# bruniss/multi-task-3d-resencoder-unet

Hardware: AMD Instinct MI355X
Metric: train patches/sec (b,c,z,y,x) ResEncM 1x128^3 (higher is better)
Workload: dtype bf16; 1 GPU; cfg2: ResEncM (6 stages, feats [32, 64, 128, 256, 512, 512], blocks [1, 3, 4, 6, 6, 6]), 1-in, heads ['sheet'], patch 128x128x128, batch 2/GPU, full train step (fwd+loss+bwd+allreduce+clip+AdamW); global_batch=2, parallelism=dp1

## Files before the change

include/rxunet.h:

```cpp
#ifndef RXUNET_H
#define RXUNET_H

#include <stddef.h>
#include <stdint.h>

#ifdef __cplusplus
extern "C" {
#endif

#define RX_OK 0
#define RX_EINVAL (-1)
#define RX_EUNSUPPORTED (-2)
#define RX_ELAUNCH (-3)
#define RX_EWORKSPACE (-4)

typedef enum { RX_F32 = 0, RX_BF16 = 1, RX_F16 = 2 } rx_dtype;
typedef enum { RX_ACT_NONE = 0, RX_ACT_SIGMOID = 1, RX_ACT_SOFTMAX = 2 } rx_head_act;

typedef struct {
  void* ptr;
  int32_t n, z, y, x, c, ld;
  int64_t cs;
} rx_act;

// ... 10 lines not shown
                  const int* taps, void* const* w_fwd, void* const* w_bwd, void* stream);

size_t rx_conv_workspace_hint(void);
int rx_conv3d_fwd(rx_dtype dt, const rx_act* x, const void* w_fwd, const float* bias, const rx_act* y,
                  const int32_t kernel[3], const int32_t stride[3], void* ws, size_t ws_bytes, void* stream);
int rx_conv3d_fwd_stats(rx_dtype dt, const rx_act* x, const void* w_fwd, const float* bias, const rx_act* y,
                        const int32_t kernel[3], const int32_t stride[3], float eps, float* stats, void* ws,
                        size_t ws_bytes, void* stream);
int rx_conv3d_bwd_data(rx_dtype dt, const rx_act* dy, const void* w_bwd, const rx_act* dx,
                       const int32_t kernel[3], const int32_t stride[3], int accumulate, void* ws,
                       size_t ws_bytes, void* stream);
int rx_conv3d_bwd_data_instats(rx_dtype dt, const rx_act* dy, const void* w_bwd, const rx_act* dx,
                               const int32_t kernel[3], const int32_t stride[3], int accumulate, const rx_act* in_y,
                               const float* in_stats, float slope, float* m12, int* fused, void* ws, size_t ws_bytes,
                               void* stream);
size_t rx_conv3d_bwd_weight_workspace(const rx_act* x, const rx_act* dy, const int32_t kernel[3]);
int rx_conv3d_bwd_weight(rx_dtype dt, const rx_act* x, const rx_act* dy, float* dw, const int32_t kernel[3],
                         const int32_t stride[3], void* ws, size_t ws_bytes, void* stream);

int rx_convT3d_fwd(rx_dtype dt, const rx_act* x, const void* w_fwd, const float* bias, const rx_act* y,
                   const int32_t stride[3], void* ws, size_t ws_bytes, void* stream);
int rx_convT3d_bwd_data(rx_dtype dt, const rx_act* dy, const void* w_bwd, const rx_act* dx,
                        const int32_t stride[3], int accumulate, void* ws, size_t ws_bytes, void* stream);
size_t rx_convT3d_bwd_weight_workspace(const rx_act* x, const rx_act* dy, const int32_t stride[3]);
int rx_convT3d_bwd_weight(rx_dtype dt, const rx_act* x, const rx_act* dy, float* dw, const int32_t stride[3],
                          void* ws, size_t ws_bytes, void* stream);

size_t rx_instnorm_stats_workspace(const rx_act* y);
int rx_instnorm_stats(rx_dtype dt, const rx_act* y, float eps, float* stats, void* ws, size_t ws_bytes,
                      void* stream);
// ... 183 lines not shown
```

multi-task-3d-resencoder-unet_amd/csrc/rx_common.h:

```cpp
#pragma once
#include <hip/hip_runtime.h>
#include <type_traits>
#include <stdint.h>
#include <stdio.h>
#include <stdlib.h>
#include <string.h>

#include "../../include/rxunet.h"

hipError_t rx_func_attr_once(const void* fn, hipFuncAttribute attr, int value);
#ifndef RX_NO_HOST_MACROS
#define hipFuncSetAttribute(fn, attr, value) rx_func_attr_once((fn), (attr), (value))
#endif

inline int rx_env_mask(const char* name) {
  const char* e = getenv(name);
  return e ? atoi(e) : 0;
}

#define RX_WAVE 64

typedef __bf16 bf16_t;
typedef _Float16 f16_t;
typedef float f32x4 __attribute__((ext_vector_type(4)));
// ... 22 lines not shown
  } while (0)

#ifndef RX_ST16
#define RX_ST16 1
#endif
__device__ inline u32x4 rx_pair16(u32x2 a, u32x2 b) {
  auto r0 = __builtin_amdgcn_permlane32_swap(a[0], b[0], false, false);
  auto r1 = __builtin_amdgcn_permlane32_swap(a[1], b[1], false, false);
  return u32x4{r0[0], r1[0], r0[1], r1[1]};
}

struct RxBwdStat {
  const rx_act* y;
  const float* stats;
  float slope;
};

#ifndef RX_ABLATION
#define RX_ABLATION 0
#endif
#define RX_ABLATE(g, bit) (RX_ABLATION && ((g).dbg & (bit)))

template <typename T>
struct Elem;
template <>
struct Elem<float> {
  static constexpr int PER16 = 4;
  __device__ static inline float to_f(float v) { return v; }
  __device__ static inline float from_f(float v) { return v; }
};
// ... 174 lines not shown
```

multi-task-3d-resencoder-unet_amd/csrc/rx_conv_halo.hip:

```cpp
#include <stdlib.h>

#include <type_traits>

#include "rx_common.h"
#include "rx_internal.h"

struct ConvHaloGeom {
  int N, Z, Y, X;
  int Ci, Co, ldi, ldo;
  long in_ss, out_ss;
  long in_cs, out_cs;
  int TZ, TY, TX, lTX, lTY;
  int HY, HX, HV, VT;
  int tz_n, ty_n, tx_n, NT;
  int order;
  int wgs_s;
  float* stat_part;
  const void* bs_y;
  const float* bs_stats;
  int bs_ldy;
  long bs_yss;
  float bs_slope;
  int accumulate, flip, dbg;
};

#define RX_CH_MAX_HV 656
#define RX_CH_XPIECES ((RX_CH_MAX_HV * 4 + 255) / 256)

__device__ inline int hswz(int row, int chunk) { return row * 4 + (chunk ^ ((row >> 2) & 3)); }

__device__ inline int lane_voxel(int l ) {
  return l < 4 ? l : l < 12 ? l + 12 : l < 16 ? l - 8 : l < 20 ? l + 8 : l < 28 ? l - 12 : l;
}

template <typename T, int BN>
__global__ __launch_bounds__(256, 2) void conv_halo_kernel(const T* __restrict__ in, const T* __restrict__ w, const float* __restrict__ bias,
                                                           T* __restrict__ out, const ConvHaloGeom g) {
// ... 540 lines not shown
        if (RX_ST16) {
#pragma unroll
          for (int pr = 0; pr < 2; ++pr)
            *reinterpret_cast<u32x4*>(op + 16 * pr + 8 * fh) = rx_pair16(piece[2 * pr], piece[2 * pr + 1]);
        }
      }
      lds_only_barrier();
    }
    if (STATS || BS) ch_stat_flush<1>(s1, s2, g.stat_part, sn, g.wgs_s * 4, sl * 4 + wave, g.Co, 0, lane);
  }
}

#define CH64_W_BYTES (9 * 64 * 64)
#define CH64_X_BYTES (648 * 64)

template <typename T, bool FLIP, bool XDMA = false, bool STATS = false, bool ACC = false, bool BSP = false, int NA = 2>
__global__ __launch_bounds__(512, 1) void conv_halo64ws_kernel(const T* __restrict__ in, const T* __restrict__ w, const float* __restrict__ bias,
                                                               T* __restrict__ out, const ConvHaloGeom g, int tiles_per_wg) {
  constexpr int P = Elem<T>::PER16;
  constexpr int KB = 4 * P;
  constexpr int TZ = 4, TY = 4, TX = 16, HY = TY + 2, HX = TX + 2, HV = 648;
  constexpr int XPIECES = (HV * 4 + 255) / 256;
  static_assert(NA == 2 || (XDMA && !BSP), "32-channel blocks: LDS-DMA variants without backward sums only");
  constexpr int BNW = 32 * NA;
  constexpr int W_BYTES = 9 * BNW * 64;
  constexpr int WINSTR = 9 * BNW / 16;
  constexpr int WPIECES = (WINSTR + 3) / 4;
  constexpr int CENTRE = HY * HX + HX + 1;
  extern __shared__ __attribute__((aligned(16))) unsigned char smem[];
  unsigned char* sWb = smem;
  unsigned char* sXb = smem + 2 * W_BYTES;

  const int tid = threadIdx.x, lane = tid & 63;
  const int wave = __builtin_amdgcn_readfirstlane(tid >> 6);
  const int lid = g.order ? rx_xcd_remap(blockIdx.y * gridDim.x + blockIdx.x, gridDim.x * gridDim.y) : blockIdx.x * gridDim.y + blockIdx.y;
  const int vb = lid / gridDim.y;
  int t_begin = vb * tiles_per_wg, t_end = min(g.NT, t_begin + tiles_per_wg);
  const int NTs = g.NT / g.N;
// ... 81 lines not shown
      }
    };
    auto commit_phase = [&](int ph) {
      if (ph % 3 == 0) {
        unsigned char* sX = sXb + ((ph / 3) & 1) * CH64_X_BYTES;
#pragma unroll
        for (int p = 0; p < XPIECES; ++p) {
          const int row = (ptid >> 2) + 64 * p;
          if (xh[p] >= 0) *reinterpret_cast<u32x4*>(sX + row * 64 + ((chunk ^ ((row >> 2) & 3)) << 4)) = xr[p];
        }
      }
    };
    if (XDMA) {
      const int bc = ptid & 7, bvg = ptid >> 3;
      float bs1[8], bs2[8], bmean[8];
      u32x4 yv[8];
      if (BSP) {
#pragma unroll
        for (int j = 0; j < 8; ++j) bs1[j] = 0.f, bs2[j] = 0.f, bmean[j] = g.bs_stats[2 * ((size_t)sn * g.Co + n0 + 8 * bc + j)];
      }
      auto bs_load_y = [&](int tile) {
        int n, z0, y0, x0;
        tile_origin(tile, n, z0, y0, x0);
        const T* yp = (const T*)g.bs_y + (long)n * g.bs_yss + n0 + 8 * bc;
#pragma unroll
        for (int p = 0; p < 8; ++p) {
          const int v = bvg + 32 * p;
          const int z = z0 + (v >> 6), y = y0 + ((v >> 4) & 3), x = x0 + (v & 15);
          yv[p] = (z < g.Z && y < g.Y && x < g.X) ? *reinterpret_cast<const u32x4*>(yp + ((long)(z * g.Y + y) * g.X + x) * g.bs_ldy) : u32x4{0u, 0u, 0u, 0u};
        }
      };
      auto bs_accumulate = [&](int tile, const unsigned char* sS) {
        int n, z0, y0, x0;
        tile_origin(tile, n, z0, y0, x0);
#pragma unroll
        for (int p = 0; p < 8; ++p) {
          const int v = bvg + 32 * p;
          const int z = z0 + (v >> 6), y = y0 + ((v >> 4) & 3), x = x0 + (v & 15);
          if (z < g.Z && y < g.Y && x < g.X) {
            const u32x4 gq = *reinterpret_cast<const u32x4*>(sS + v * 144 + bc * 16);
#pragma unroll
            for (int j = 0; j < 8; ++j) {
              float gg = Elem<T>::to_f(reinterpret_cast<const T*>(&gq)[j]);
              const float yc = Elem<T>::to_f(reinterpret_cast<const T*>(&yv[p])[j]) - bmean[j];
              if (!(yc > 0.f)) gg *= g.bs_slope;
              bs1[j] += gg;
              bs2[j] += gg * yc;
            }
          }
        }
      };
      if (nphase > 0) {
        dma_weights(0);
        dma_halo(0);
        asm volatile("s_waitcnt vmcnt(0)" ::: "memory");
      }
      lds_only_barrier();
      int pit = 0, pending = -1;
      const unsigned char* pendS = nullptr;
      for (int ph = 0; ph < nphase; ++ph) {
        const bool tile_end = pit == ppt - 1;
        if (ph + 1 < nphase) {
          dma_weights(ph + 1);
          if (ph + 2 < nphase && (ph + 2) % 3 == 0) {
            dma_halo(ph + 2);
            if (pw == 0)
              asm volatile("s_waitcnt vmcnt(11)" ::: "memory");
            else
              asm volatile("s_waitcnt vmcnt(10)" ::: "memory");
          } else {
            if (BSP && pending >= 0) {
              bs_accumulate(pending, pendS);
              pending = -1;
            }
            if (BSP && tile_end) bs_load_y(t_begin + ph / ppt);
            asm volatile("s_waitcnt vmcnt(0)" ::: "memory");
          }
        } else if (BSP) {
          bs_load_y(t_begin + ph / ppt);
          asm volatile("s_waitcnt vmcnt(0)" ::: "memory");
        }
        lds_only_barrier();
        if (++pit == ppt) {
          pit = 0;
          if (BSP) {
            lds_only_barrier();
            pending = t_begin + ph / ppt;
            pendS = sXb + ((ph / 3) & 1) * CH64_X_BYTES;
          }
        }
      }
      if (BSP) {
        if (pending >= 0) bs_accumulate(pending, pendS);
#pragma unroll
        for (int j = 0; j < 8; ++j) {
          float u = bs1[j], v = bs2[j];
#pragma unroll
          for (int o = 8; o < 64; o <<= 1) {
            u += __shfl_xor(u, o, 64);
            v += __shfl_xor(v, o, 64);
          }
          bs1[j] = u, bs2[j] = v;
        }
        if (pl < 8) {
          float* p0 = g.stat_part + ((size_t)(sn * (g.wgs_s * 4) + sl * 4 + pw) * 2) * g.Co + n0 + 8 * pl;
#pragma unroll
          for (int j = 0; j < 8; ++j) p0[j] = bs1[j], p0[g.Co + j] = bs2[j];
        }
// ... 154 lines not shown
                else if (decltype(RA)::value) f += Elem<T>::to_f(reinterpret_cast<const T*>(&old2)[i]);
                vals[i] = Elem<T>::from_f(f);
                if (STATS) {
                  const float r = Elem<T>::to_f(vals[i]);
                  s1[a][4 * g4 + i] += r;
                  s2[a][4 * g4 + i] += r * r;
                }
              }
              if (BSP) *reinterpret_cast<u32x2*>(sS + v * SROW + co * 2) = *reinterpret_cast<u32x2*>(vals);
              else if (!RX_ABLATE(g, 16) || vals[0] == (T)12345.f) *reinterpret_cast<u32x2*>(op + cm) = *reinterpret_cast<u32x2*>(vals);
            }
        };
        RX_EPI_DISPATCH(bias != nullptr, !ACC && g.accumulate != 0, epi);
      }
      lds_only_barrier();
      if (BSP) {
        int t2 = tid;
        asm volatile("" : "+v"(t2));
        const int ry = t2 >> 7, rx = (t2 >> 3) & 15, c = t2 & 7;
        T* gp = out + (long)n * g.out_ss + ((long)(z0 * g.Y + y0 + ry) * g.X + x0 + rx) * g.ldo + n0 + (c >> 2) * g.out_cs + (c & 3) * 8;
        const unsigned char* lp = sS + (t2 >> 3) * SROW + c * 16;
        const bool okx = x0 + rx < g.X;
#pragma unroll
        for (int p = 0; p < 8; ++p) {
          const int zz = p >> 1, yy = 2 * (p & 1);
          if (okx && z0 + zz < g.Z && y0 + ry + yy < g.Y)
            *reinterpret_cast<u32x4*>(gp + ((long)(zz * g.Y + yy) * g.X) * g.ldo) = *reinterpret_cast<const u32x4*>(lp + p * 32 * SROW);
        }
      }
      ++ph;
    }
// ... 13 lines not shown
  const int per = (NTs + wgs_s - 1) / wgs_s;
  wgs_s = (NTs + per - 1) / per;
  wgs = wgs_s * g.N;
  const_cast<ConvHaloGeom&>(g).wgs_s = wgs_s;
  dim3 grid(wgs, cob);
#define RX_64WS(...)                                                                                                                   \
  do {                                                                                                                                 \
    (void)hipFuncSetAttribute(reinterpret_cast<const void*>(&conv_halo64ws_kernel<T, __VA_ARGS__>), hipFuncAttributeMaxDynamicSharedMemorySize, (int)lds); \
    hipLaunchKernelGGL((conv_halo64ws_kernel<T, __VA_ARGS__>), grid, dim3(512), lds, st, (const T*)in, (const T*)w, bias, (T*)out, g, per); \
  } while (0)
  const bool dma_ok = (long)g.N * g.in_ss * 2 < 0x7fffff00L;
  if (dma_ok && g.stat_part && !g.flip && !g.bs_y) {
    RX_64WS(false, true, true);
    return;
  }
  if (dma_ok && g.bs_y && g.stat_part && g.flip && !((uintptr_t)out & 15) && g.ldo % 8 == 0 && g.out_cs % 8 == 0 && !((uintptr_t)g.bs_y & 15) &&
      g.bs_ldy % 8 == 0) {
    if (g.accumulate) RX_64WS(true, true, false, true, true);
    else RX_64WS(true, true, false, false, true);
    return;
  }
  const_cast<ConvHaloGeom&>(g).bs_y = nullptr;
  const_cast<ConvHaloGeom&>(g).stat_part = nullptr;
  if (dma_ok && g.accumulate && g.flip) RX_64WS(true, true, false, true);
  else if (dma_ok && g.flip) RX_64WS(true, true);
  else if (dma_ok) RX_64WS(false, true);
  else if (g.flip) RX_64WS(true, false);
  else RX_64WS(false, false);
#undef RX_64WS
}

template <typename T>
static bool ch32ws_launch(hipStream_t st, const void* in, const void* w, const float* bias, void* out, const ConvHaloGeom& g) {
  const size_t lds = (size_t)2 * (9 * 32 * 64 + CH64_X_BYTES);
// ... 128 lines not shown
  g.tz_n = (g.Z + TZ - 1) / TZ, g.ty_n = (g.Y + TY - 1) / TY, g.tx_n = (g.X + TX - 1) / TX;
  g.NT = g.N * g.tz_n * g.ty_n * g.tx_n;
  g.accumulate = accumulate, g.flip = flip;
  g.order = 1;
  static const int dbg = rx_env_mask("RX_DBG");
  g.dbg = dbg;
  int BN = (g.Co % 64 == 0) ? 64 : 32;
  if (BN == 64 && (long)g.NT * (g.Co / 64) < 256) BN = 32;
  if ((in->cs || out->cs) && (long)g.NT * (g.Co / BN) < 192) RX_FAIL(RX_EUNSUPPORTED, "conv_halo: planar-concat operand on a layer too small for the halo kernels");
  if ((long)g.NT * (g.Co / BN) < 192) return 0;
  dim3 grid(g.NT, g.Co / BN);
  if (BN == 32 && TZ == 4 && TY == 4 && TX == 16 && dt != RX_F32 && g.Ci == 32 && g.Co == 32 && g.NT >= 512) {
    rx_note_kernel("conv_halo32p_kernel");
    if (in->cs || out->cs) RX_FAIL(RX_EUNSUPPORTED, "conv_halo32p: planar-concat operand");
    const bool room = stat_part && stat_chunks && (size_t)g.N * 1024 * 2 * g.Co * sizeof(float) <= stat_bytes;
    const bool fuse32 = room && ((!flip && !accumulate && !bs) || (flip && bs));
    g.stat_part = fuse32 ? stat_part : nullptr;
    if (fuse32 && bs) {
      g.bs_y = bs->y->ptr, g.bs_ldy = bs->y->ld, g.bs_yss = rx_act_voxels(bs->y) * (long)bs->y->ld;
      g.bs_stats = bs->stats, g.bs_slope = bs->slope;
    }
    if (dt == RX_BF16)
      ch32p_launch<bf16_t>(st, in->ptr, w, bias, out->ptr, g);
    else
      ch32p_launch<f16_t>(st, in->ptr, w, bias, out->ptr, g);
    hipError_t e4 = hipGetLastError();
    if (e4 != hipSuccess) {
      rx_set_error("conv_halo32p: %s", hipGetErrorString(e4));
      return RX_ELAUNCH;
    }
    if (fuse32) *stat_chunks = g.wgs_s * 4;
// ... 39 lines not shown
      return RX_ELAUNCH;
    }
    if (fuse32n) *stat_chunks = NTs32 * 4;
    return 1;
  }
  if (g.Co % 64 == 0 && TZ == 4 && TY == 4 && TX == 16 && dt != RX_F32 && (long)g.NT * (g.Co / 64) >= 256) {
    if (in->cs) RX_FAIL(RX_EUNSUPPORTED, "conv_halo64ws: planar-concat input");
    rx_note_kernel("conv_halo64ws_kernel");
    const bool room64 = stat_part && stat_chunks && (size_t)g.N * 1024 * 2 * g.Co * sizeof(float) <= stat_bytes;
    const bool fuse64 = room64 && !flip && !accumulate && !bs;
    const bool fuse64b = room64 && flip && bs;
    g.stat_part = (fuse64 || fuse64b) ? stat_part : nullptr;
    if (fuse64b) {
      g.bs_y = bs->y->ptr, g.bs_ldy = bs->y->ld, g.bs_yss = rx_act_voxels(bs->y) * (long)bs->y->ld;
      g.bs_stats = bs->stats, g.bs_slope = bs->slope;
    }
    if (dt == RX_BF16)
      ch64ws_launch<bf16_t>(st, in->ptr, w, bias, out->ptr, g);
    else
      ch64ws_launch<f16_t>(st, in->ptr, w, bias, out->ptr, g);
    hipError_t e5 = hipGetLastError();
    if (e5 != hipSuccess) {
      rx_set_error("conv_halo64ws: %s", hipGetErrorString(e5));
      return RX_ELAUNCH;
    }
    if (fuse64 && g.stat_part) *stat_chunks = g.wgs_s * 4;
    if (fuse64b && g.bs_y && g.stat_part) *stat_chunks = g.wgs_s * 4;
    g.stat_part = nullptr, g.bs_y = nullptr;
    return 1;
  }
// ... 16 lines not shown
```

multi-task-3d-resencoder-unet_amd/csrc/rx_igemm.hip:

```cpp
#include <stdlib.h>

#include "rx_common.h"
#include "rx_internal.h"


struct IgemmPhase {
  int Qz, Qy, Qx, Vq;
  int opz, opy, opx;
  int tap0, ntaps;
  int mtile0, mtiles;
  long slab_off;
};

struct IgemmGeom {
  int Zi, Yi, Xi, Ci, ldi;
  long in_ss;
  int isz, isy, isx;
  int Zo, Yo, Xo, Co, ldo;
  long out_ss;
  int osz, osy, osx;
  int accumulate, ksplit, nph, total_mtiles;
  IgemmPhase ph[8];
  RxTap taps[RX_MAX_TAPS];
};
// ... 530 lines not shown
    RxBwdStat bs{in_y, in_stats, slope};
    int chunks = 0;
    rc = rx_conv_halo_try(dt, dy, w_bwd, nullptr, dx, 1, accumulate, (hipStream_t)stream, (float*)ws, wsb, &chunks, &bs);
    if (rc < 0) return rc;
    if (rc == 1) {
      if (chunks > 0) {
        rx_inbwd_fused_finalize_launch((const float*)ws, dx->n, chunks, dx->c, (double)rx_act_voxels(dx), in_stats, m12, (hipStream_t)stream);
        hipError_t e = hipGetLastError();
        if (e != hipSuccess) RX_FAIL(RX_ELAUNCH, "rx_conv3d_bwd_data_instats(finalize): %s", hipGetErrorString(e));
        *fused = 1;
      }
      return RX_OK;
    }
  }
  return rx_conv3d_bwd_data(dt, dy, w_bwd, dx, kernel, stride, accumulate, ws, wsb, stream);
}

extern "C" int rx_conv3d_fwd_stats(rx_dtype dt, const rx_act* x, const void* w_fwd, const float* bias, const rx_act* y,
                                   const int32_t kernel[3], const int32_t stride[3], float eps, float* stats, void* ws, size_t wsb,
                                   void* stream) {
  RX_RECORD(stream, [=, x_ = RxActV(x), y_ = RxActV(y), kernel_ = RxI3V(kernel), stride_ = RxI3V(stride)](void* s) { return rx_conv3d_fwd_stats(dt, x_.p(), w_fwd, bias, y_.p(), kernel_.v, stride_.v, eps, stats, ws, wsb, s); });
  if (!rx_act_ok_planar(x) || !rx_act_ok(y) || !w_fwd || !stats || !ws) RX_FAIL(RX_EINVAL, "rx_conv3d_fwd_stats: bad arguments");
  int rc = check13(kernel, stride, "rx_conv3d_fwd_stats");
  if (rc) return rc;
  if (is_333_s1(kernel, stride) && y->n == x->n && y->z == x->z && y->y == x->y && y->x == x->x) {
    int chunks = 0;
    rc = rx_conv_halo_try(dt, x, w_fwd, bias, y, 0, 0, (hipStream_t)stream, (float*)ws, wsb, &chunks, nullptr);
    if (rc < 0) return rc;
    if (rc == 1 && chunks > 0) {
      rx_stats_finalize_launch((const float*)ws, y->n, chunks, y->c, (double)rx_act_voxels(y), eps, stats, (hipStream_t)stream);
// ... 171 lines not shown
```

multi-task-3d-resencoder-unet_amd/engine/lib.py:

```python
import ctypes
import os
from ctypes import POINTER, c_char_p, c_double, c_float, c_int, c_int32, c_long, c_size_t, c_void_p

import torch

_HERE = os.path.dirname(os.path.abspath(__file__))
LIB_PATH = os.environ.get("RX_LIBRARY") or os.path.join(os.path.dirname(_HERE), "csrc", "librxunet.so")

RX_F32, RX_BF16, RX_F16 = 0, 1, 2
RX_ACT_NONE, RX_ACT_SIGMOID, RX_ACT_SOFTMAX = 0, 1, 2
DTYPE_CODE = {torch.float32: RX_F32, torch.bfloat16: RX_BF16, torch.float16: RX_F16}
RX_SW_U8, RX_SW_U16, RX_SW_F32 = 0, 1, 2
RX_SW_SCALE, RX_SW_ZSCORE = 0, 1
RX_SW_BLEND_AVERAGE, RX_SW_BLEND_UNIT, RX_SW_BLEND_NONE = 0, 1, 2
RX_SW_CAST_U8, RX_SW_CAST_U16 = 0, 1
RX_AUG_PW_NONE, RX_AUG_PW_AFFINE, RX_AUG_PW_PLANE, RX_AUG_PW_NOISE = 0, 1, 2, 3
RX_AUG_G3_NONE, RX_AUG_G3_FILTER, RX_AUG_G3_DOWNSCALE = 0, 1, 2
RX_AUG_MAX_K, RX_AUG_MAX_BOXES = 21, 4
RX_LOSS_BCE_LOGITS, RX_LOSS_BCE_PROB, RX_LOSS_MSE = 0, 1, 2
RX_REDUCE_MEAN, RX_REDUCE_SUM = 0, 1


class RxError(RuntimeError):
    pass
# ... 15 lines not shown

_SIGNATURES = {
    "rx_abi_version": (c_int, []),
    "rx_last_error": (c_char_p, []),
    "rx_device_arch_ok": (c_int, []),
    "rx_last_conv_kernel": (c_char_p, []),
    "rx_pack_conv_weight": (c_int, [c_int, c_void_p, c_int, c_int, c_int, c_void_p, c_void_p, c_void_p]),
    "rx_pack_convT_weight": (c_int, [c_int, c_void_p, c_int, c_int, c_int, c_void_p, c_void_p, c_void_p]),
    "rx_pack_multi": (c_int, [c_int, c_int, c_void_p, c_void_p, c_void_p, c_void_p, c_void_p, c_void_p, c_void_p, c_void_p]),
    "rx_conv_workspace_hint": (c_size_t, []),
    "rx_conv3d_fwd": (c_int, [c_int, _P, c_void_p, c_void_p, _P, I3, I3, c_void_p, c_size_t, c_void_p]),
    "rx_conv3d_fwd_stats": (c_int, [c_int, _P, c_void_p, c_void_p, _P, I3, I3, c_float, c_void_p, c_void_p, c_size_t, c_void_p]),
    "rx_conv3d_bwd_data": (c_int, [c_int, _P, c_void_p, _P, I3, I3, c_int, c_void_p, c_size_t, c_void_p]),
    "rx_conv3d_bwd_data_instats": (c_int, [c_int, _P, c_void_p, _P, I3, I3, c_int, _P, c_void_p, c_float, c_void_p, POINTER(c_int),
                                           c_void_p, c_size_t, c_void_p]),
    "rx_instnorm_act_bwd_apply": (c_int, [c_int, _P, _P, c_void_p, _P, c_float, c_void_p, _P, _P, c_int, c_void_p]),
    "rx_conv3d_bwd_weight_workspace": (c_size_t, [_P, _P, I3]),
    "rx_conv3d_bwd_weight": (c_int, [c_int, _P, _P, c_void_p, I3, I3, c_void_p, c_size_t, c_void_p]),
    "rx_convT3d_fwd": (c_int, [c_int, _P, c_void_p, c_void_p, _P, I3, c_void_p, c_size_t, c_void_p]),
    "rx_convT3d_bwd_data": (c_int, [c_int, _P, c_void_p, _P, I3, c_int, c_void_p, c_size_t, c_void_p]),
    "rx_convT3d_bwd_weight_workspace": (c_size_t, [_P, _P, I3]),
    "rx_convT3d_bwd_weight": (c_int, [c_int, _P, _P, c_void_p, I3, c_void_p, c_size_t, c_void_p]),
    "rx_instnorm_stats_workspace": (c_size_t, [_P]),
    "rx_instnorm_stats": (c_int, [c_int, _P, c_float, c_void_p, c_void_p, c_size_t, c_void_p]),
    "rx_instnorm_act_fwd": (c_int, [c_int, _P, c_void_p, _P, _P, c_float, c_void_p]),
    "rx_instnorm_stats_mask": (c_int, [c_void_p, c_void_p, c_int, c_void_p]),
    "rx_instnorm_fwd": (c_int, [c_int, _P, c_float, c_void_p, _P, _P, c_float, c_void_p, c_size_t, c_void_p]),
    "rx_instnorm_act_bwd": (c_int, [c_int, _P, _P, c_void_p, _P, c_float, _P, _P, c_int, c_void_p, c_size_t,
                                    c_void_p]),
    "rx_instnorm_act_bwd_res": (c_int, [c_int, _P, _P, c_void_p, _P, c_float, _P, I3, _P, _P, c_void_p, c_size_t, c_void_p]),
# ... 132 lines not shown
```

multi-task-3d-resencoder-unet_amd/engine/ops.py:

```python
from ctypes import byref, c_void_p

import numpy as np
import torch

from . import lib as _l
from .lib import I3, RxAct, check, load, stream_ptr

_WS = {}
_PROF = None


def set_profiler(p):
    global _PROF
    _PROF = p


class LaunchProfiler:

    def __init__(self):
        self.pending = []
        self.groups = {}
        self.pending_hbm = []
        self.hbm = {}

# ... 292 lines not shown
    if _PROF is None:
        return go()
    n = dy.dims[0]
    _PROF.run("dgrad:" + LaunchProfiler.igemm_name(dx.voxels, dx.c), 2.0 * n * dy.voxels * dy.c * dx.c * _taps(kernel), 1, go)


def conv3d_bwd_data_instats(dy, w_bwd, dx, kernel, stride, accumulate, in_y, in_stats, slope, m12, ws=None):
    from ctypes import c_int
    ws = workspace() if ws is None else ws
    fused = c_int(0)

    def go():
        check(load().rx_conv3d_bwd_data_instats(_code(dy.dtype), byref(dy.desc()), _ptr(w_bwd), byref(dx.desc()), I3(*kernel),
                                                I3(*stride), int(accumulate), byref(in_y.desc()), _ptr(in_stats), float(slope),
                                                _ptr(m12), byref(fused), *_ws_args(ws), stream_ptr()), "rx_conv3d_bwd_data_instats")
    if _PROF is None:
        go()
    else:
        n = dx.dims[0]
        _PROF.run("dgrad:" + LaunchProfiler.igemm_name(dx.voxels, dx.c), 2.0 * n * dx.voxels * dx.c * dy.c * _taps(kernel), 1, go)
    return bool(fused.value)


def instnorm_act_bwd_apply(g, y, stats, out, dy, m12, slope=0.01, d_residual=None, accumulate_residual=False):
    check(load().rx_instnorm_act_bwd_apply(_code(y.dtype), byref(g.desc()), byref(y.desc()), _ptr(stats),
                                           byref(out.desc()) if out is not None else None, float(slope), _ptr(m12),
                                           byref(dy.desc()),
                                           byref(d_residual.desc()) if d_residual is not None else None,
                                           int(accumulate_residual), stream_ptr()), "rx_instnorm_act_bwd_apply")

# ... 422 lines not shown
```

multi-task-3d-resencoder-unet_amd/engine/plan.py:

```python
import contextlib
import os
from dataclasses import dataclass
from typing import Callable, ClassVar, Dict, List, NamedTuple, Optional

import torch
from torch import nn

from . import lib as _l
from . import ops
from .ops import Act


class UnsupportedConfig(NotImplementedError):
    pass


_SIDE_STREAMS: Dict[str, "torch.cuda.Stream"] = {}


def side_stream(device):
    key = str(device)
    st = _SIDE_STREAMS.get(key)
    if st is None:
        st = _SIDE_STREAMS[key] = torch.cuda.Stream(device=device)
# ... 82 lines not shown


@dataclass(eq=False)
class ConvRec:
    kind: ClassVar[str] = "conv"
    x: AT
    y: AT
    pk: dict
    b: Optional[torch.Tensor]
    widx: int
    bidx: Optional[int]
    kernel: list
    stride: list
    stats_to: Optional["InactRec"] = None
    instats_for: Optional["InactRec"] = None


@dataclass(eq=False)
class ConvTRec:
    kind: ClassVar[str] = "convT"
    x: AT
    y: AT
    pk: dict
    b: Optional[torch.Tensor]
    widx: int
    bidx: Optional[int]
    stride: list
    cat: AT


# ... 4 lines not shown
    stats: torch.Tensor
    eps: float
    res: Optional[AT]
    out: AT
    slope: float
    gate: Optional[Gate]
    drop: Optional[Drop]
    stats_done: bool = False
    pool_to: Optional["PoolRec"] = None
    head_to: Optional["HeadRec"] = None
    head_src: Optional["HeadRec"] = None
    head_dw_fused: bool = False
    m12: Optional[torch.Tensor] = None
    m12_valid: bool = False
    m12x: Optional[torch.Tensor] = None


@dataclass(eq=False)
class PoolRec:
    kind: ClassVar[str] = "pool"
    x: AT
    y: AT
    stride: list
    fused: bool = False


@dataclass(eq=False)
class CopyRec:
    kind: ClassVar[str] = "copy"
    x: AT
# ... 743 lines not shown
        gres, acc = None, False
        if res is not None and res.needs_grad:
            gres, acc = self._claim_grad(res, r)
        plain16 = r.gate is None and res is None and self.dtype != torch.float32 and _above_single_launch(out.act)
        last = out.last_writer
        if plain16 and isinstance(last, HeadRec):
            heads = [h for h in tape if h.kind == "head" and h.x is out]
            if len(heads) == 1 and heads[0].k <= 4:
                r.head_src, last.dx_fused = heads[0], True
                if heads[0].fwd_fused and heads[0].w is self.params[heads[0].widx]:
                    r.head_dw_fused, last.dw_fused = True, True
        if (plain16 and isinstance(last, ConvRec) and out.act.full_buffer and out.act.root is None and out.act.c % 32 == 0
                and _halo_x_ok(out.act)):
            r.m12 = torch.empty((self.B, out.act.c, 2), dtype=torch.float32, device=self.device)
            last.instats_for = r
        if r.gate is not None:
            return [self._bwd_inact_gated(r, gout, dy, gres, acc)]
        pend, out.pool_pending = out.pool_pending, None
        if gres is not None and not acc and _above_single_launch(y.act):
            return [self._bwd_inact_res(r, gout, dy, gres, pend)]
        steps = []
        if pend is not None:
            steps.append(lambda: ops.avgpool_bwd(pend.gy, pend.gx, pend.stride, True))
        return steps + [self._bwd_inact_plain(r, gout, dy, gres, acc)]

    def _bwd_inact_gated(self, r, gout, dy, gres, acc):
        g = r.gate

        def step():
            self._before_dy_write(dy)
            if g.se is None and g.scale_now is None:
                ops.instnorm_act_bwd(gout, r.y.act, r.stats, r.out.act if (r.slope != 1.0 and r.res is not None) else None, dy,
                                     r.slope, gres, acc)
                return
            grads = [self._new_grad(j) for j in g.se.idx] if g.se is not None else [None] * 4
            ops.se_gate_bwd(gout, r.y.act, r.stats, r.out.act, r.slope, g.se_args(), g.pooled, g.hidden, g.gate, g.mult, g.dadd,
                            g.m12, *grads, path_scale=g.scale_now)
            ops.instnorm_gate_act_bwd(gout, r.y.act, r.stats, r.out.act, r.slope, g.mult, g.dadd, g.m12, g.keep_x, dy, gres, acc)
            if g.se is not None:
                for j in g.se.idx:
                    self._grad_done(j)
        if g.se is not None:
            self.grad_order += g.se.idx
        return step

    def _bwd_inact_res(self, r, gout, dy, gres, pend):
        def step():
            self._before_dy_write(dy)
            ops.instnorm_act_bwd_res(gout, r.y.act, r.stats, r.out.act, dy, gres, r.slope,
                                     pool_dy=pend.gy if pend is not None else None,
                                     pool_stride=pend.stride if pend is not None else (1, 1, 1))
        return step

    def _bwd_inact_plain(self, r, gout, dy, gres, acc):
        mask_out = r.out.act if (r.slope != 1.0 and r.res is not None) else None
        hs = r.head_src

        def step():
            self._before_dy_write(dy)
            dl = self._dlogits.get(hs.name) if hs is not None else None
            if dl is not None and r.head_dw_fused:
                dw, db = self._new_grad(hs.widx), self._new_grad(hs.bidx)
                ops.instnorm_act_bwd_head(dl, hs.w.view(hs.k, -1), r.y.act, r.stats, dy, r.slope, dw=dw.view(hs.k, -1), db=db)
# ... 11 lines not shown
            else:
                ops.instnorm_act_bwd(gout, r.y.act, r.stats, mask_out, dy, r.slope, gres, acc)
        return step

    def _bwd_conv(self, r, tape, i):
        dy = r.y.gact

        def wlaunch(dw, ws):
            if r.kind == "stem":
                ops.stem_conv_bwd_weight(self._x, dy, dw, r.kernel, ws)
            elif "wgrad" not in self._skip:
                ops.conv3d_bwd_weight(r.x.act, dy, dw, r.kernel, r.stride, ws)
        steps = [self._wgrad_step(r, dy, wlaunch)]
        if r.kind == "conv" and r.x.needs_grad:
            gx, acc = self._claim_grad(r.x, r)
            if r.x.act.full_buffer:
                self._cat_written[r.x.act.key] = True

            def dstep():
                if "dgrad" in self._skip:
                    return
                ia = r.instats_for
                if ia is None:
                    ops.conv3d_bwd_data(dy, r.pk["w_bwd"], gx, r.kernel, r.stride, acc)
                else:
                    ia.m12_valid = ops.conv3d_bwd_data_instats(dy, r.pk["w_bwd"], gx, r.kernel, r.stride, acc, ia.y.act, ia.stats,
                                                               ia.slope, ia.m12)
            steps.append(dstep)
        return steps

    def _bwd_convT(self, r: ConvTRec, tape, i):
        if not self._view_written(r.y):
            raise RuntimeError("plan bug: concat gradient not initialised before the transposed conv")
        gy = self._cat_grad(r)
        gx, acc = self._claim_grad(r.x, r)
        wstep = self._wgrad_step(r, gy, lambda dw, ws: ops.convT3d_bwd_weight(r.x.act, gy, dw, r.stride, ws))

        def step():
            wstep()
# ... 464 lines not shown
```

Baseline: 117.9 patches/s.

## Fuse residual-branch instnorm backward sums into accumulating 3x3x3 dgrad kernel

Adds a residual mode to the 64-channel halo dgrad kernel. When the kernel accumulates into the residual gradient buffer, it now also applies the leaky-ReLU mask from the block output, writes the pre-norm gradient to a separate buffer, and accumulates the instnorm backward sums. The planner routes eligible residual instnorm layers through this path, so the later instnorm backward only applies the precomputed sums and does not re-read and reduce the gradients. The cost is extra loads and stores in the conv epilogue, higher register pressure, and tighter eligibility conditions.

Result: no change. 117.8 patches/s (median of 2 runs) (-0.1%).

```diff
diff --git a/include/rxunet.h b/include/rxunet.h
--- a/include/rxunet.h
+++ b/include/rxunet.h
@@ -48,6 +48,10 @@
                                const int32_t kernel[3], const int32_t stride[3], int accumulate, const rx_act* in_y,
                                const float* in_stats, float slope, float* m12, int* fused, void* ws, size_t ws_bytes,
                                void* stream);
+int rx_conv3d_bwd_data_instats_res(rx_dtype dt, const rx_act* dy, const void* w_bwd, const rx_act* dx,
+                                   const int32_t kernel[3], const int32_t stride[3], const rx_act* in_y,
+                                   const float* in_stats, const rx_act* in_out, float slope, const rx_act* d_residual,
+                                   float* m12, int* fused, void* ws, size_t ws_bytes, void* stream);
 size_t rx_conv3d_bwd_weight_workspace(const rx_act* x, const rx_act* dy, const int32_t kernel[3]);
 int rx_conv3d_bwd_weight(rx_dtype dt, const rx_act* x, const rx_act* dy, float* dw, const int32_t kernel[3],
                          const int32_t stride[3], void* ws, size_t ws_bytes, void* stream);
diff --git a/multi-task-3d-resencoder-unet_amd/csrc/rx_common.h b/multi-task-3d-resencoder-unet_amd/csrc/rx_common.h
--- a/multi-task-3d-resencoder-unet_amd/csrc/rx_common.h
+++ b/multi-task-3d-resencoder-unet_amd/csrc/rx_common.h
@@ -60,6 +60,8 @@
   const rx_act* y;
   const float* stats;
   float slope;
+  const rx_act* out = nullptr;
+  const rx_act* gp = nullptr;
 };
 
 #ifndef RX_ABLATION
diff --git a/multi-task-3d-resencoder-unet_amd/csrc/rx_conv_halo.hip b/multi-task-3d-resencoder-unet_amd/csrc/rx_conv_halo.hip
--- a/multi-task-3d-resencoder-unet_amd/csrc/rx_conv_halo.hip
+++ b/multi-task-3d-resencoder-unet_amd/csrc/rx_conv_halo.hip
@@ -21,6 +21,8 @@
   int bs_ldy;
   long bs_yss;
   float bs_slope;
+  const void* bs_out;
+  void* bs_gp;
   int accumulate, flip, dbg;
 };
 
@@ -591,7 +593,7 @@
 #define CH64_W_BYTES (9 * 64 * 64)
 #define CH64_X_BYTES (648 * 64)
 
-template <typename T, bool FLIP, bool XDMA = false, bool STATS = false, bool ACC = false, bool BSP = false, int NA = 2>
+template <typename T, bool FLIP, bool XDMA = false, bool STATS = false, bool ACC = false, bool BSP = false, int NA = 2, bool RES = false>
 __global__ __launch_bounds__(512, 1) void conv_halo64ws_kernel(const T* __restrict__ in, const T* __restrict__ w, const float* __restrict__ bias,
                                                                T* __restrict__ out, const ConvHaloGeom g, int tiles_per_wg) {
   constexpr int P = Elem<T>::PER16;
@@ -599,6 +601,7 @@
   constexpr int TZ = 4, TY = 4, TX = 16, HY = TY + 2, HX = TX + 2, HV = 648;
   constexpr int XPIECES = (HV * 4 + 255) / 256;
   static_assert(NA == 2 || (XDMA && !BSP), "32-channel blocks: LDS-DMA variants without backward sums only");
+  static_assert(!RES || (BSP && ACC && XDMA && NA == 2), "residual mode: an accumulating LDS-DMA launch with backward sums");
   constexpr int BNW = 32 * NA;
   constexpr int W_BYTES = 9 * BNW * 64;
   constexpr int WINSTR = 9 * BNW / 16;
@@ -710,7 +713,7 @@
     if (XDMA) {
       const int bc = ptid & 7, bvg = ptid >> 3;
       float bs1[8], bs2[8], bmean[8];
-      u32x4 yv[8];
+      u32x4 yv[8], ov[RES ? 8 : 1];
       if (BSP) {
 #pragma unroll
         for (int j = 0; j < 8; ++j) bs1[j] = 0.f, bs2[j] = 0.f, bmean[j] = g.bs_stats[2 * ((size_t)sn * g.Co + n0 + 8 * bc + j)];
@@ -718,20 +721,29 @@
       auto bs_load_y = [&](int tile) {
         int n, z0, y0, x0;
         tile_origin(tile, n, z0, y0, x0);
-        const T* yp = (const T*)g.bs_y + (long)n * g.bs_yss + n0 + 8 * bc;
+        int bvg2 = bvg;
+        if (RES) asm volatile("" : "+v"(bvg2));
+        const long base = (long)n * g.bs_yss + n0 + 8 * bc;
+        const T* yp = (const T*)g.bs_y + base;
+        const T* op = (const T*)g.bs_out + base;
 #pragma unroll
         for (int p = 0; p < 8; ++p) {
-          const int v = bvg + 32 * p;
+          const int v = bvg2 + 32 * p;
           const int z = z0 + (v >> 6), y = y0 + ((v >> 4) & 3), x = x0 + (v & 15);
-          yv[p] = (z < g.Z && y < g.Y && x < g.X) ? *reinterpret_cast<const u32x4*>(yp + ((long)(z * g.Y + y) * g.X + x) * g.bs_ldy) : u32x4{0u, 0u, 0u, 0u};
+          const bool ok = z < g.Z && y < g.Y && x < g.X;
+          const long vo = ((long)(z * g.Y + y) * g.X + x) * g.bs_ldy;
+          yv[p] = ok ? *reinterpret_cast<const u32x4*>(yp + vo) : u32x4{0u, 0u, 0u, 0u};
+          if (RES) ov[RES ? p : 0] = ok ? *reinterpret_cast<const u32x4*>(op + vo) : u32x4{0u, 0u, 0u, 0u};
         }
       };
       auto bs_accumulate = [&](int tile, const unsigned char* sS) {
         int n, z0, y0, x0;
         tile_origin(tile, n, z0, y0, x0);
+        int bvg2 = bvg;
+        if (RES) asm volatile("" : "+v"(bvg2));
 #pragma unroll
         for (int p = 0; p < 8; ++p) {
-          const int v = bvg + 32 * p;
+          const int v = bvg2 + 32 * p;
           const int z = z0 + (v >> 6), y = y0 + ((v >> 4) & 3), x = x0 + (v & 15);
           if (z < g.Z && y < g.Y && x < g.X) {
             const u32x4 gq = *reinterpret_cast<const u32x4*>(sS + v * 144 + bc * 16);
@@ -739,11 +751,29 @@
             for (int j = 0; j < 8; ++j) {
               float gg = Elem<T>::to_f(reinterpret_cast<const T*>(&gq)[j]);
               const float yc = Elem<T>::to_f(reinterpret_cast<const T*>(&yv[p])[j]) - bmean[j];
-              if (!(yc > 0.f)) gg *= g.bs_slope;
+              if (RES) {
+                if (!(Elem<T>::to_f(reinterpret_cast<const T*>(&ov[RES ? p : 0])[j]) > 0.f)) gg *= g.bs_slope;
+                const T w = Elem<T>::from_f(gg);
+                reinterpret_cast<T*>(&ov[RES ? p : 0])[j] = w;
+                gg = Elem<T>::to_f(w);
+              } else if (!(yc > 0.f)) gg *= g.bs_slope;
               bs1[j] += gg;
               bs2[j] += gg * yc;
             }
           }
+        }
+      };
+      auto bs_store_gp = [&](int tile) {
+        int n, z0, y0, x0;
+        tile_origin(tile, n, z0, y0, x0);
+        int bvg2 = bvg;
+        if (RES) asm volatile("" : "+v"(bvg2));
+        T* gp = (T*)g.bs_gp + (long)n * g.bs_yss + n0 + 8 * bc;
+#pragma unroll
+        for (int p = 0; p < 8; ++p) {
+          const int v = bvg2 + 32 * p;
+          const int z = z0 + (v >> 6), y = y0 + ((v >> 4) & 3), x = x0 + (v & 15);
+          if (z < g.Z && y < g.Y && x < g.X) *reinterpret_cast<u32x4*>(gp + ((long)(z * g.Y + y) * g.X + x) * g.bs_ldy) = ov[RES ? p : 0];
         }
       };
       if (nphase > 0) {
@@ -765,12 +795,14 @@
             else
               asm volatile("s_waitcnt vmcnt(10)" ::: "memory");
           } else {
+            const int done = pending;
             if (BSP && pending >= 0) {
               bs_accumulate(pending, pendS);
               pending = -1;
             }
             if (BSP && tile_end) bs_load_y(t_begin + ph / ppt);
             asm volatile("s_waitcnt vmcnt(0)" ::: "memory");
+            if (RES && done >= 0) bs_store_gp(done);
           }
         } else if (BSP) {
           bs_load_y(t_begin + ph / ppt);
@@ -787,7 +819,10 @@
         }
       }
       if (BSP) {
-        if (pending >= 0) bs_accumulate(pending, pendS);
+        if (pending >= 0) {
+          bs_accumulate(pending, pendS);
+          if (RES) bs_store_gp(pending);
+        }
 #pragma unroll
         for (int j = 0; j < 8; ++j) {
           float u = bs1[j], v = bs2[j];
@@ -972,7 +1007,7 @@
         RX_EPI_DISPATCH(bias != nullptr, !ACC && g.accumulate != 0, epi);
       }
       lds_only_barrier();
-      if (BSP) {
+      if (BSP && !RES) {
         int t2 = tid;
         asm volatile("" : "+v"(t2));
         const int ry = t2 >> 7, rx = (t2 >> 3) & 15, c = t2 & 7;
@@ -1016,10 +1051,16 @@
     RX_64WS(false, true, true);
     return;
   }
-  if (dma_ok && g.bs_y && g.stat_part && g.flip && !((uintptr_t)out & 15) && g.ldo % 8 == 0 && g.out_cs % 8 == 0 && !((uintptr_t)g.bs_y & 15) &&
-      g.bs_ldy % 8 == 0) {
+  const bool bsp_ok = dma_ok && g.bs_y && g.stat_part && g.flip && !((uintptr_t)out & 15) && g.ldo % 8 == 0 && g.out_cs % 8 == 0 &&
+                      !((uintptr_t)g.bs_y & 15) && g.bs_ldy % 8 == 0;
+  if (bsp_ok && !g.bs_out) {
     if (g.accumulate) RX_64WS(true, true, false, true, true);
     else RX_64WS(true, true, false, false, true);
+    return;
+  }
+  if (bsp_ok && g.bs_out && g.accumulate && !((uintptr_t)g.bs_out & 15) && !((uintptr_t)g.bs_gp & 15)) {
+    rx_note_kernel("conv_halo64ws_kernel<res>");
+    RX_64WS(true, true, false, true, true, 2, true);
     return;
   }
   const_cast<ConvHaloGeom&>(g).bs_y = nullptr;
@@ -1178,7 +1219,7 @@
     rx_note_kernel("conv_halo32p_kernel");
     if (in->cs || out->cs) RX_FAIL(RX_EUNSUPPORTED, "conv_halo32p: planar-concat operand");
     const bool room = stat_part && stat_chunks && (size_t)g.N * 1024 * 2 * g.Co * sizeof(float) <= stat_bytes;
-    const bool fuse32 = room && ((!flip && !accumulate && !bs) || (flip && bs));
+    const bool fuse32 = room && ((!flip && !accumulate && !bs) || (flip && bs && !bs->out));
     g.stat_part = fuse32 ? stat_part : nullptr;
     if (fuse32 && bs) {
       g.bs_y = bs->y->ptr, g.bs_ldy = bs->y->ld, g.bs_yss = rx_act_voxels(bs->y) * (long)bs->y->ld;
@@ -1248,6 +1289,8 @@
     if (fuse64b) {
       g.bs_y = bs->y->ptr, g.bs_ldy = bs->y->ld, g.bs_yss = rx_act_voxels(bs->y) * (long)bs->y->ld;
       g.bs_stats = bs->stats, g.bs_slope = bs->slope;
+      if (bs->out && bs->out->ld == bs->y->ld && bs->gp->ld == bs->y->ld) g.bs_out = bs->out->ptr, g.bs_gp = bs->gp->ptr;
+      else if (bs->out) g.bs_y = nullptr;
     }
     if (dt == RX_BF16)
       ch64ws_launch<bf16_t>(st, in->ptr, w, bias, out->ptr, g);
diff --git a/multi-task-3d-resencoder-unet_amd/csrc/rx_igemm.hip b/multi-task-3d-resencoder-unet_amd/csrc/rx_igemm.hip
--- a/multi-task-3d-resencoder-unet_amd/csrc/rx_igemm.hip
+++ b/multi-task-3d-resencoder-unet_amd/csrc/rx_igemm.hip
@@ -568,6 +568,38 @@
     }
   }
   return rx_conv3d_bwd_data(dt, dy, w_bwd, dx, kernel, stride, accumulate, ws, wsb, stream);
+}
+
+extern "C" int rx_conv3d_bwd_data_instats_res(rx_dtype dt, const rx_act* dy, const void* w_bwd, const rx_act* dx, const int32_t kernel[3],
+                                              const int32_t stride[3], const rx_act* in_y, const float* in_stats, const rx_act* in_out,
+                                              float slope, const rx_act* d_residual, float* m12, int* fused, void* ws, size_t wsb,
+                                              void* stream) {
+  RX_RECORD(stream, [=, dy_ = RxActV(dy), dx_ = RxActV(dx), kernel_ = RxI3V(kernel), stride_ = RxI3V(stride), in_y_ = RxActV(in_y), in_out_ = RxActV(in_out), d_residual_ = RxActV(d_residual)](void* s) { int fused_dummy = 0; return rx_conv3d_bwd_data_instats_res(dt, dy_.p(), w_bwd, dx_.p(), kernel_.v, stride_.v, in_y_.p(), in_stats, in_out_.p(), slope, d_residual_.p(), m12, &fused_dummy, ws, wsb, s); });
+  if (!fused || !m12 || !in_stats || !rx_act_ok(in_y) || !rx_act_ok(in_out) || !rx_act_ok(d_residual) || !ws)
+    RX_FAIL(RX_EINVAL, "rx_conv3d_bwd_data_instats_res: bad arguments");
+  *fused = 0;
+  if (!rx_act_ok(dy) || !rx_act_ok(dx) || !w_bwd) RX_FAIL(RX_EINVAL, "rx_conv3d_bwd_data_instats_res: bad arguments");
+  int rc = check13(kernel, stride, "rx_conv3d_bwd_data_instats_res");
+  if (rc) return rc;
+  auto same = [&](const rx_act* a) { return a->n == dx->n && a->z == dx->z && a->y == dx->y && a->x == dx->x && a->c == dx->c; };
+  if (!same(in_y) || !same(in_out) || !same(d_residual)) RX_FAIL(RX_EINVAL, "rx_conv3d_bwd_data_instats_res: geometry mismatch");
+  if (d_residual->ptr == dx->ptr) RX_FAIL(RX_EINVAL, "rx_conv3d_bwd_data_instats_res: d_residual and dx must be different buffers");
+  if (is_333_s1(kernel, stride) && dx->z == dy->z && dx->y == dy->y && dx->x == dy->x && dt != RX_F32) {
+    RxBwdStat bs{in_y, in_stats, slope, in_out, d_residual};
+    int chunks = 0;
+    rc = rx_conv_halo_try(dt, dy, w_bwd, nullptr, dx, 1, 1, (hipStream_t)stream, (float*)ws, wsb, &chunks, &bs);
+    if (rc < 0) return rc;
+    if (rc == 1) {
+      if (chunks > 0) {
+        rx_inbwd_fused_finalize_launch((const float*)ws, dx->n, chunks, dx->c, (double)rx_act_voxels(dx), in_stats, m12, (hipStream_t)stream);
+        hipError_t e = hipGetLastError();
+        if (e != hipSuccess) RX_FAIL(RX_ELAUNCH, "rx_conv3d_bwd_data_instats_res(finalize): %s", hipGetErrorString(e));
+        *fused = 1;
+      }
+      return RX_OK;
+    }
+  }
+  return rx_conv3d_bwd_data(dt, dy, w_bwd, dx, kernel, stride, 1, ws, wsb, stream);
 }
 
 extern "C" int rx_conv3d_fwd_stats(rx_dtype dt, const rx_act* x, const void* w_fwd, const float* bias, const rx_act* y,
diff --git a/multi-task-3d-resencoder-unet_amd/engine/lib.py b/multi-task-3d-resencoder-unet_amd/engine/lib.py
--- a/multi-task-3d-resencoder-unet_amd/engine/lib.py
+++ b/multi-task-3d-resencoder-unet_amd/engine/lib.py
@@ -53,6 +53,8 @@
     "rx_conv3d_bwd_data": (c_int, [c_int, _P, c_void_p, _P, I3, I3, c_int, c_void_p, c_size_t, c_void_p]),
     "rx_conv3d_bwd_data_instats": (c_int, [c_int, _P, c_void_p, _P, I3, I3, c_int, _P, c_void_p, c_float, c_void_p, POINTER(c_int),
                                            c_void_p, c_size_t, c_void_p]),
+    "rx_conv3d_bwd_data_instats_res": (c_int, [c_int, _P, c_void_p, _P, I3, I3, _P, c_void_p, _P, c_float, _P, c_void_p,
+                                               POINTER(c_int), c_void_p, c_size_t, c_void_p]),
     "rx_instnorm_act_bwd_apply": (c_int, [c_int, _P, _P, c_void_p, _P, c_float, c_void_p, _P, _P, c_int, c_void_p]),
     "rx_conv3d_bwd_weight_workspace": (c_size_t, [_P, _P, I3]),
     "rx_conv3d_bwd_weight": (c_int, [c_int, _P, _P, c_void_p, I3, I3, c_void_p, c_size_t, c_void_p]),
diff --git a/multi-task-3d-resencoder-unet_amd/engine/ops.py b/multi-task-3d-resencoder-unet_amd/engine/ops.py
--- a/multi-task-3d-resencoder-unet_amd/engine/ops.py
+++ b/multi-task-3d-resencoder-unet_amd/engine/ops.py
@@ -330,6 +330,24 @@
         check(load().rx_conv3d_bwd_data_instats(_code(dy.dtype), byref(dy.desc()), _ptr(w_bwd), byref(dx.desc()), I3(*kernel),
                                                 I3(*stride), int(accumulate), byref(in_y.desc()), _ptr(in_stats), float(slope),
                                                 _ptr(m12), byref(fused), *_ws_args(ws), stream_ptr()), "rx_conv3d_bwd_data_instats")
+    if _PROF is None:
+        go()
+    else:
+        n = dx.dims[0]
+        _PROF.run("dgrad:" + LaunchProfiler.igemm_name(dx.voxels, dx.c), 2.0 * n * dx.voxels * dx.c * dy.c * _taps(kernel), 1, go)
+    return bool(fused.value)
+
+
+def conv3d_bwd_data_instats_res(dy, w_bwd, dx, kernel, stride, in_y, in_stats, in_out, slope, d_residual, m12, ws=None):
+    from ctypes import c_int
+    ws = workspace() if ws is None else ws
+    fused = c_int(0)
+
+    def go():
+        check(load().rx_conv3d_bwd_data_instats_res(_code(dy.dtype), byref(dy.desc()), _ptr(w_bwd), byref(dx.desc()), I3(*kernel),
+                                                    I3(*stride), byref(in_y.desc()), _ptr(in_stats), byref(in_out.desc()),
+                                                    float(slope), byref(d_residual.desc()), _ptr(m12), byref(fused),
+                                                    *_ws_args(ws), stream_ptr()), "rx_conv3d_bwd_data_instats_res")
     if _PROF is None:
         go()
     else:
diff --git a/multi-task-3d-resencoder-unet_amd/engine/plan.py b/multi-task-3d-resencoder-unet_amd/engine/plan.py
--- a/multi-task-3d-resencoder-unet_amd/engine/plan.py
+++ b/multi-task-3d-resencoder-unet_amd/engine/plan.py
@@ -120,6 +120,7 @@
     stride: list
     stats_to: Optional["InactRec"] = None
     instats_for: Optional["InactRec"] = None
+    dgrad_acc: bool = False
 
 
 @dataclass(eq=False)
@@ -154,6 +155,7 @@
     m12: Optional[torch.Tensor] = None
     m12_valid: bool = False
     m12x: Optional[torch.Tensor] = None
+    gres_from_dgrad: Optional[Act] = None
 
 
 @dataclass(eq=False)
@@ -927,15 +929,28 @@
                 and _halo_x_ok(out.act)):
             r.m12 = torch.empty((self.B, out.act.c, 2), dtype=torch.float32, device=self.device)
             last.instats_for = r
+        pend, out.pool_pending = out.pool_pending, None
+        if r.gate is None and gres is not None and not acc and pend is None:
+            self._fuse_dgrad_res_sums(r, tape, i, gres)
         if r.gate is not None:
             return [self._bwd_inact_gated(r, gout, dy, gres, acc)]
-        pend, out.pool_pending = out.pool_pending, None
         if gres is not None and not acc and _above_single_launch(y.act):
             return [self._bwd_inact_res(r, gout, dy, gres, pend)]
         steps = []
         if pend is not None:
             steps.append(lambda: ops.avgpool_bwd(pend.gy, pend.gx, pend.stride, True))
         return steps + [self._bwd_inact_plain(r, gout, dy, gres, acc)]
+
+    def _fuse_dgrad_res_sums(self, r, tape, i, gres):
+        out, last = r.out, r.out.last_writer
+        if ("dgrad_res_sums" in self._skip or self.dtype == torch.float32 or not _above_single_launch(out.act)
+                or not isinstance(last, ConvRec) or not last.dgrad_acc or i + 1 >= len(tape) or tape[i + 1] is not last
+                or list(last.kernel) != [3, 3, 3] or list(last.stride) != [1, 1, 1]
+                or not (out.act.full_buffer and out.act.root is None and out.act.c % 64 == 0 and _halo_x_ok(out.act))
+                or not (gres.full_buffer and gres.root is None and r.y.act.full_buffer and r.y.act.root is None)):
+            return
+        r.m12 = torch.empty((self.B, out.act.c, 2), dtype=torch.float32, device=self.device)
+        last.instats_for, r.gres_from_dgrad = r, gres
 
     def _bwd_inact_gated(self, r, gout, dy, gres, acc):
         g = r.gate
@@ -960,6 +975,10 @@
     def _bwd_inact_res(self, r, gout, dy, gres, pend):
         def step():
             self._before_dy_write(dy)
+            if r.m12_valid:
+                r.m12_valid = False
+                ops.instnorm_act_bwd_apply(gres, r.y.act, r.stats, None, dy, r.m12, 1.0)
+                return
             ops.instnorm_act_bwd_res(gout, r.y.act, r.stats, r.out.act, dy, gres, r.slope,
                                      pool_dy=pend.gy if pend is not None else None,
                                      pool_stride=pend.stride if pend is not None else (1, 1, 1))
@@ -1001,6 +1020,7 @@
         steps = [self._wgrad_step(r, dy, wlaunch)]
         if r.kind == "conv" and r.x.needs_grad:
             gx, acc = self._claim_grad(r.x, r)
+            r.dgrad_acc = acc
             if r.x.act.full_buffer:
                 self._cat_written[r.x.act.key] = True
 
@@ -1010,6 +1030,9 @@
                 ia = r.instats_for
                 if ia is None:
                     ops.conv3d_bwd_data(dy, r.pk["w_bwd"], gx, r.kernel, r.stride, acc)
+                elif ia.gres_from_dgrad is not None:
+                    ia.m12_valid = ops.conv3d_bwd_data_instats_res(dy, r.pk["w_bwd"], gx, r.kernel, r.stride, ia.y.act, ia.stats,
+                                                                   ia.out.act, ia.slope, ia.gres_from_dgrad, ia.m12)
                 else:
                     ia.m12_valid = ops.conv3d_bwd_data_instats(dy, r.pk["w_bwd"], gx, r.kernel, r.stride, acc, ia.y.act, ia.stats,
                                                                ia.slope, ia.m12)
```
